# federicomegler/sq-learn

Measured on AMD Instinct MI355X. Metric: q-means fit samples/sec (Lloyd samples*iterations/s, delta-means + tomography noise), higher is better.
Workload: dtype fp32; 1 GPU; model=q-means k=1024 delta=0.5 (10000000 x 256 synthetic), global_batch=10000000, seq_len=256, parallelism=dp1

## Files before the change

sq_learn_amd/csrc/estep_f32.hip:

```cpp
#include "common.h"
#include "band.h"
#include "f16_tile.h"

namespace sq {

constexpr int kMaxCand = 16;

#ifndef SQ_SPLIT_ACC_ALL
#define SQ_SPLIT_ACC_ALL 1
#endif
template <int KSD, int TOP = 2>
__global__ void __launch_bounds__(256, 1) estep_f32_kernel(
    const float* __restrict__ X, const _Float16* __restrict__ C, const float* __restrict__ xn,
    int* __restrict__ labels, float* __restrict__ mind, long long* __restrict__ ovf_rows,
    int* __restrict__ ovf_count, double* __restrict__ part, long long n, int k_pad, float alpha,
    float inv_alpha2, float delta_s, RngKey key, long long row_offset, int ovf_cap,
    const long long* __restrict__ rlist, const int* __restrict__ rcount,
    const float* __restrict__ cmax2_p, long long* __restrict__ mrows, int* __restrict__ mcand,
    int* __restrict__ multi_count, unsigned char* __restrict__ xflag, long long mcap) {
  const float Cm = cmax2_p ? sqrtf(*cmax2_p) * (1.0f + 0x1p-16f) : 0.0f;
  constexpr bool SPLIT_ACC = SQ_SPLIT_ACC_ALL || TOP == 3;
  constexpr float kEps3 =
      SPLIT_ACC ? (3.0f * 0x1p-22f + (KSD * 16 + 18.0f) * 0x1p-24f + 2.0f * KSD * 16 * 0x1p-34f) *
                      1.0625f
// ... 906 lines not shown
  for (int p = 0; p < PER && act; ++p) {
    if (act & (1ull << p)) {
      rlist[pos++] = c0 + (long long)p * 256 + tid;
      act &= ~(1ull << p);
    }
  }
  int mpos = base_m + (ex >> 16);
  for (int p = 0; p < PER && rec; ++p) {
    if (rec & (1ull << p)) {
      mrows[mpos++] = c0 + (long long)p * 256 + tid;
      rec &= ~(1ull << p);
    }
  }
  int bpos = base_b + before_b + incl_b - mine_b;
  for (int p = 0; p < PER && recb; ++p) {
    if (recb & (1ull << p)) {
      mrows_b[bpos++] = c0 + (long long)p * 256 + tid;
      recb &= ~(1ull << p);
    }
  }
}

struct MultiRec {
  GapRec* rec = nullptr;
  int* mflag = nullptr;
  int it_now = 0, it_lo = 0;
  int ring = 0;
  const _Float16* dsh = nullptr;
  const float* dq = nullptr;
  long long dsh_stride = 0;
  long long* mrows_b = nullptr;
  int* count_b = nullptr;
  int* n_done = nullptr;
};
static thread_local MultiRec g_mrec;
struct Ovf2 {
  void* rows = nullptr;
  int* count = nullptr;
};
static thread_local Ovf2 g_ovf2;
extern "C" int sq_set_overflow2(void* rows, void* count) {
  g_ovf2.rows = rows;
  g_ovf2.count = (int*)count;
  return (rows != nullptr) != (count != nullptr) ? (int)hipErrorInvalidValue : 0;
}
extern "C" int sq_multi_records(void* rec, void* mflag, int it_now, int it_lo, int ring,
                                const void* dsh, const void* dq, long long dsh_stride,
                                void* mrows_b, void* count_b, void* n_done) {
  g_mrec.rec = (GapRec*)rec;
  g_mrec.mflag = (int*)mflag;
  g_mrec.it_now = it_now;
  g_mrec.it_lo = it_lo;
  g_mrec.ring = ring;
  g_mrec.dsh = (const _Float16*)dsh;
  g_mrec.dq = (const float*)dq;
  g_mrec.dsh_stride = dsh_stride;
  g_mrec.mrows_b = (long long*)mrows_b;
  g_mrec.count_b = (int*)count_b;
  g_mrec.n_done = (int*)n_done;
  return (rec && (it_now < 1 || it_lo < 1 || it_lo > it_now || ring < 2 || ring > 16 || !mflag ||
                  !dsh || !dq || !mrows_b || !count_b))
             ? (int)hipErrorInvalidValue
             : 0;
}

extern "C" int sq_bounds_filter(const void* labels, void* ub, void* lb, const void* shift,
                                const void* smax, long long n, double delta, void* rlist,
                                void* rcount, const void* mflag, void* mrows, void* multi_count,
                                const void* cc, const void* fidx, int nf, int k, void* stream,
                                void* corr, void* rec_count) {
  if (n <= 0) return 0;
  if (!mflag || !mrows || !multi_count) return (int)hipErrorInvalidValue;
  if (nf < 0 || nf > 64 || (nf > 0 && (!cc || !fidx || k <= nf))) return (int)hipErrorInvalidValue;
  hipStream_t st = (hipStream_t)stream;
  static long long resident = 0;
  if (resident == 0) {
    int dev = 0, cus = 0, per_cu = 0;
    hipGetDevice(&dev);
    hipDeviceGetAttribute(&cus, hipDeviceAttributeMultiprocessorCount, dev);
    hipOccupancyMaxActiveBlocksPerMultiprocessor(&per_cu, (const void*)bounds_filter_kernel<32>,
                                                 256, 0);
    resident = (long long)(cus > 0 ? cus : 256) * (per_cu > 0 ? per_cu : 4);
  }
  auto pick = [&](int per) { return (n + per * 256LL - 1) / (per * 256LL) <= resident; };
  static const int per_env = [] {
    const char* e = getenv("SQ_BF_PER");
    return e ? atoi(e) : 0;
  }();
  int per = pick(8) ? 8 : pick(16) ? 16 : pick(20) ? 20 : pick(32) ? 32 : 64;
  if (per_env == 4 || per_env == 8 || per_env == 16 || per_env == 20 || per_env == 32 ||
      per_env == 64)
    per = per_env;
// ... 376 lines not shown
  acc = __builtin_amdgcn_fdot2(__builtin_bit_cast(gs_h2, a.x), __builtin_bit_cast(gs_h2, b.x), acc,
                               false);
  acc = __builtin_amdgcn_fdot2(__builtin_bit_cast(gs_h2, a.y), __builtin_bit_cast(gs_h2, b.y), acc,
                               false);
  acc = __builtin_amdgcn_fdot2(__builtin_bit_cast(gs_h2, a.z), __builtin_bit_cast(gs_h2, b.z), acc,
                               false);
  acc = __builtin_amdgcn_fdot2(__builtin_bit_cast(gs_h2, a.w), __builtin_bit_cast(gs_h2, b.w), acc,
                               false);
  return acc;
}
__device__ __forceinline__ float gs_dot(const uint2 a, const uint2 b, float acc) {
  acc = __builtin_amdgcn_fdot2(__builtin_bit_cast(gs_h2, a.x), __builtin_bit_cast(gs_h2, b.x), acc,
                               false);
  acc = __builtin_amdgcn_fdot2(__builtin_bit_cast(gs_h2, a.y), __builtin_bit_cast(gs_h2, b.y), acc,
                               false);
  return acc;
}
__device__ __forceinline__ uint4 gs_zero(uint4) { return make_uint4(0u, 0u, 0u, 0u); }
template <int CTRL>
__device__ __forceinline__ float gs_dpp_add(float v) {
  return v + __int_as_float(__builtin_amdgcn_update_dpp(0, __float_as_int(v), CTRL, 0xF, 0xF,
                                                         false));
}
__device__ __forceinline__ uint2 gs_zero(uint2) { return make_uint2(0u, 0u); }

template <int DX>
__global__ void __launch_bounds__(256) gap_screen_kernel(
    const _Float16* __restrict__ Xh, const float* __restrict__ xn,
    const long long* __restrict__ mrows_b, const int* __restrict__ count_b,
    const _Float16* __restrict__ dsh, long long dsh_stride, const float* __restrict__ dq,
    long long dq_stride, float inv_alpha, float delta, int* __restrict__ labels,
    GapRec* __restrict__ rec, int* __restrict__ mflag, int it_now, int ring, int rebase_age,
    long long* __restrict__ mrows, int* __restrict__ multi_count, long long cap,
    int* __restrict__ n_done) {
  constexpr int LPR = 32;
  using VT = typename std::conditional<DX % 256 == 0, uint4, uint2>::type;
  constexpr int HV = (int)sizeof(VT) / 2;
  constexpr int V = DX / (LPR * HV);
  static_assert(DX % 128 == 0 && V >= 1, "gap screen: d_pad multiple of 128");
  const int lane = threadIdx.x & 63;
  const int sub = lane & (LPR - 1);
  const bool hi = lane >= LPR;
  const long long cnt = min((long long)*count_b, cap);
  const long long gw = (long long)blockIdx.x * (blockDim.x >> 6) + (threadIdx.x >> 6);
  const long long nw = (long long)gridDim.x * (blockDim.x >> 6);
  const long long nblk = (cnt + 63) / 64;
  const float sub_err = sqrtf((float)DX) * 0x1p-25f * inv_alpha;
  constexpr float gam = (float)(DX + 16) * 0x1p-24f;
  uint32_t done_cnt = 0;
  auto rl = [](int v, int l) -> int { return __builtin_amdgcn_readlane(v, l); };
  auto rlf = [](float v, int l) -> float {
    return __int_as_float(__builtin_amdgcn_readlane(__float_as_int(v), l));
  };
  for (long long blk = gw; blk < nblk; blk += nw) {
    const long long e = blk * 64 + lane;
    const bool live = e < cnt;
    const long long g = mrows_b[live ? e : cnt - 1];
    const int base_it = mflag[g] - 2;
    const int rslot = base_it % ring, age = it_now - base_it;
    const float4* rp = reinterpret_cast<const float4*>(rec + g);
    const float4 r0 = rp[0], r1 = rp[1];
    const float xq = xn[g];
    const unsigned id0 = __float_as_uint(r1.z), id1 = __float_as_uint(r1.w);
    const int c_r = (int)(id0 >> 30) + 1, slot = (int)((id0 >> 14) & 3u);
    int jc[kGapCand];
    jc[0] = (int)(id0 & 0x3FFFu);
    jc[1] = (int)((id0 >> 16) & 0x3FFFu);
    jc[2] = (int)(id1 & 0x3FFFu);
    jc[3] = (int)((id1 >> 16) & 0x3FFFu);
    const float* dqs = dq + (size_t)rslot * dq_stride;
    float4 d0[kGapCand];
    float inv[kGapCand];
#pragma unroll
    for (int c = 0; c < kGapCand; ++c) {
      d0[c] = reinterpret_cast<const float4*>(dqs)[2 * jc[c]];
      inv[c] = dqs[8 * jc[c] + 4];
    }
    float y[kGapCand] = {0.0f, 0.0f, 0.0f, 0.0f};
    constexpr int NB = 4;
    VT xv[NB][V], sv[NB][kGapCand][V];
    int pcm[NB];
    auto issue = [&](int p, int b) {
// ... 85 lines not shown
    float gm = gn[0];
#pragma unroll
    for (int c = 1; c < kGapCand; ++c)
      if (gn[c] < gm) {
        gm = gn[c];
        m = c;
      }
    bool done = live && c_r >= 2 && slot < c_r && err < 0.25f * delta + 1.0f;
    float gmx = 0.0f;
#pragma unroll
    for (int c = 0; c < kGapCand; ++c)
      if (c < c_r && c != m) {
        done = done && (gn[c] - gm > delta + 2.0f * err);
        gmx = fmaxf(gmx, gn[c]);
      }
    if (done && (m != slot || age >= rebase_age)) {
      const float da_n = da + gm;
      float err_n =
          (m == slot ? err : 2.0f * err) + 0x1p-22f * (gmx + fabsf(da_n) + fabsf(gm));
      err_n *= 1.0f + 0x1p-20f;
      float gr[kGapCand];
#pragma unroll
      for (int c = 0; c < kGapCand; ++c) gr[c] = c < c_r ? gn[c] - gm : 0.0f;
      float4* wp = reinterpret_cast<float4*>(rec + g);
      wp[0] = make_float4(da_n, err_n, gr[0], gr[1]);
      wp[1] = make_float4(gr[2], gr[3],
                          __uint_as_float((id0 & ~(3u << 14)) | (unsigned)m << 14),
                          __uint_as_float(id1));
      if (m != slot) labels[g] = jc[0] * (m == 0) + jc[1] * (m == 1) + jc[2] * (m == 2) +
                                 jc[3] * (m == 3);
      mflag[g] = it_now + 2;
    }
    const bool fwd = live && !done;
    const unsigned long long fm = __ballot(fwd);
    if (fm) {
      int fb = 0;
      if (lane == 0) fb = atomicAdd(multi_count, __popcll(fm));
      fb = __shfl(fb, 0, 64);
      const long long se = (long long)fb + __popcll(fm & ((1ull << lane) - 1ull));
      if (fwd && se < cap) mrows[se] = g;
    }
    done_cnt += __popcll(__ballot(done));
  }
  if (n_done && lane == 0 && done_cnt) atomicAdd(n_done, (int)done_cnt);
}

__global__ void __launch_bounds__(256) shift_operand_kernel(
    const float* __restrict__ Cprev, const float* __restrict__ Cnew, int ldc, int d, int d_pad,
    int k, double alpha, float* __restrict__ snap, _Float16* __restrict__ dsh,
    float* __restrict__ dq, int snew, unsigned valid) {
  const int lane = threadIdx.x & 63;
  const int j = blockIdx.x * 4 + (threadIdx.x >> 6);
  const int sl = blockIdx.y;
  if (j >= k || !((valid >> sl) & 1u)) return;
  const size_t rs = (size_t)sl * k + j;
  const float* cn = Cnew + (size_t)j * ldc;
  float* sn = snap + rs * d_pad;
  const bool fresh = sl == snew;
  const float* co = fresh ? Cprev + (size_t)j * ldc : sn;
  double amax = 0.0;
  for (int f = lane; f < d; f += 64) amax = fmax(amax, fabs((double)cn[f] - (double)co[f]));
#pragma unroll
  for (int o = 32; o > 0; o >>= 1) amax = fmax(amax, __shfl_xor(amax, o, 64));
  int ex2 = 0;
  if (amax > 0.0) frexp(amax, &ex2);
  const double beta = amax > 0.0 ? ldexp(1.0, 14 - ex2) : 1.0;
  double q = 0.0, nrm = 0.0, nd = 0.0, e2 = 0.0;
  for (int f = lane; f < d_pad; f += 64) {
    const float a32 = f < d ? co[f] : 0.0f;
    const double a = (double)a32, b = f < d ? (double)cn[f] : 0.0;
    const double sft = b - a;
    const _Float16 h = (_Float16)(float)(beta * sft);
    dsh[rs * d_pad + f] = h;
    if (fresh) sn[f] = a32;
    const double r = sft - (double)h / beta;
    q += sft * (b + a);
// ... 243 lines not shown
                       (const long long*)rlist, (const int*)rcount, (float*)ub, (float*)lb,
                       (int*)mflag);
  };
  static const bool list_rs1 = [] {
    const char* e = getenv("SQ_X64_LIST_RS1");
    return !(e && e[0] == '0');
  }();
  if (rlist && (list_rs == 1 || (list_rs == 0 && list_rs1)))
    go(std::integral_constant<int, 1>{});
  else
    go(std::integral_constant<int, X64RowSets<KSD>::value>{});
  int rc = (int)hipGetLastError();
  if (rc) return rc;
  const long long rblocks = (n / 16 + 63) / 64;
  const unsigned rgrid = (unsigned)(rblocks < 4096 ? (rblocks > 0 ? rblocks : 1) : 4096);
  if (xflag && g_mrec.rec && ub) {
    if constexpr (KSD * 16 % 128 == 0) {
      static long long gres = 0;
      if (gres == 0) {
        int dev = 0, cus = 0, per_cu = 0;
        hipGetDevice(&dev);
        hipDeviceGetAttribute(&cus, hipDeviceAttributeMultiprocessorCount, dev);
        hipOccupancyMaxActiveBlocksPerMultiprocessor(
            &per_cu, (const void*)gap_screen_kernel<KSD * 16>, 256, 0);
        gres = (long long)(cus > 0 ? cus : 256) * (per_cu > 0 ? per_cu : 2);
      }
      const unsigned bgrid = (unsigned)min(max(rblocks, 1LL), gres);
      hipLaunchKernelGGL(gap_screen_kernel<KSD * 16>, dim3(bgrid), dim3(256), 0, st,
                         (const _Float16*)Xh, (const float*)xn, g_mrec.mrows_b, g_mrec.count_b,
                         g_mrec.dsh, g_mrec.dsh_stride, g_mrec.dq,
                         g_mrec.dsh_stride / (KSD * 16) * 8, 1.0f / alpha, (float)delta,
                         (int*)labels, g_mrec.rec, g_mrec.mflag, g_mrec.it_now, g_mrec.ring,
                         max(1, g_mrec.ring / 2), (long long*)mrows, (int*)multi_count, n,
                         g_mrec.n_done);
    }
  }
  if (xflag) {
    static int sgrid = 0, sil = 0;
    if (sgrid == 0) {
      const char* ei = getenv("SQ_SCREEN_IL");
      sil = ei ? atoi(ei) : 0;
      const char* e = getenv("SQ_SCREEN_GRID");
      sgrid = e ? atoi(e) : 1024;
      if (sgrid <= 0) sgrid = 4096;
    }
    const unsigned fgrid2 = (unsigned)(rblocks < sgrid ? (rblocks > 0 ? rblocks : 1) : sgrid);
    auto fk = ub ? recheck_fast_kernel<KSD * 16, SQ_SCREEN_LPR, true>
                 : recheck_fast_kernel<KSD * 16, SQ_SCREEN_LPR, false>;
    hipLaunchKernelGGL(fk, dim3(fgrid2), dim3(256), 0, st, (const float*)X, (const float*)Cm,
                       (const long long*)mrows, (const int*)mcand, (const int*)multi_count,
                       (int*)labels, (float*)mind, n, delta, (float*)ub, (unsigned char*)xflag,
                       sil, g_mrec.rec, g_mrec.mflag, g_mrec.it_now, key, row_offset,
                       (float*)corr);
  }
  if (!defer_rows)
    hipLaunchKernelGGL(recheck_rows_kernel<KSD * 16>, dim3(rgrid), dim3(256), 0, st,
                       (const float*)X, (const float*)Cm, (const long long*)mrows,
                       (const int*)mcand, (const int*)multi_count, (int*)labels, (float*)mind, n,
                       delta, key, row_offset, (float*)corr, (float*)ub,
                       (const unsigned char*)xflag);
  return (int)hipGetLastError();
}

extern "C" {

int sq_estep_f32(const void* X, const void* C, const void* xn, void* labels, void* mind,
                 void* ovf_rows, void* ovf_count, void* part, int part_cap, void* inertia,
// ... 151 lines not shown
```

sq_learn_amd/csrc/module.cpp:

```cpp
#define PY_SSIZE_T_CLEAN
#include <Python.h>
#include <hip/hip_runtime.h>

extern "C" {
__attribute__((weak)) int sq_trunc_normal_add(void*, int, long long, double, unsigned, unsigned, unsigned, unsigned,
                        unsigned long long, void*);
__attribute__((weak)) int sq_philox_normal(void*, int, long long, double, double, unsigned, unsigned, unsigned, unsigned,
                     unsigned long long, void*);
__attribute__((weak)) int sq_philox_uniform(void*, long long, unsigned, unsigned, unsigned, unsigned, unsigned long long,
                      void*);
__attribute__((weak)) int sq_ae_batch(const void*, const void*, void*, long long, int, unsigned, unsigned, unsigned,
                unsigned, unsigned long long, void*);
__attribute__((weak)) int sq_pe_batch(const void*, const void*, void*, long long, unsigned, unsigned, unsigned, unsigned,
                unsigned long long, void*);
__attribute__((weak)) int sq_tomography(const void*, int, int, const void*, int, int, const void*,
                                        void*, void*, int, unsigned, unsigned, unsigned, unsigned,
                                        long long, void*, double);
__attribute__((weak)) int sq_mnom_segments(const void*, long long, const void*, long long,
                                           long long, const void*, void*, long long, unsigned,
                                           unsigned, unsigned, unsigned, const void*, int, void*);
__attribute__((weak)) int sq_bounds_filter(const void*, void*, void*, const void*, const void*,
                                           long long, double, void*, void*, const void*, void*,
                                           void*, const void*, const void*, int, int, void*, void*,
                                           void*);
__attribute__((weak)) int sq_multi_records(void*, void*, int, int, int, const void*, const void*,
                                           long long, void*, void*, void*);
__attribute__((weak)) int sq_set_overflow2(void*, void*);
__attribute__((weak)) int sq_shift_operand(const void*, const void*, int, int, int, int, double,
                                           void*, void*, void*, int, int, unsigned, void*);
__attribute__((weak)) int sq_fast_centroids(void*, const void*, const void*, int, int, int, void*,
                                            void*, void*, void*);
__attribute__((weak)) int sq_xtx(const void*, int, long long, const void*, int, const void*, int,
                                 long long, const void*, int, long long, int, int, void*, void*,
                                 int, void*);
__attribute__((weak)) int sq_xtx_geometry(int, int, int, int*, int*, int*);
__attribute__((weak)) int sq_xw(const void*, int, long long, const void*, long long, int,
                                const void*, long long, int, int, void*, int, long long, void*);
__attribute__((weak)) int sq_ipe_fused(const void*, long long, const void*, const void*,
                                       const void*, const void*, const void*, void*, void*,
                                       long long, int, int, int, int, double, int, unsigned,
                                       unsigned, unsigned, unsigned, unsigned, unsigned, unsigned,
                                       unsigned, unsigned, unsigned, unsigned, unsigned, long long,
                                       int, void*, void*, void*, const void*, const void*,
                                       long long, const void*, const void*);
__attribute__((weak)) int sq_ipe16(int, const long long*, const double*, void*);
__attribute__((weak)) int sq_kmpp_batch(int, const long long*, void*);
__attribute__((weak)) int sq_centroid_delta(const void*, const void*, const void*, void*, void*,
                                            void*, long long, int, int, int, int, void*, void*,
                                            void*, void*);
__attribute__((weak)) int sq_centroid_delta_lists(const void*, const void*, const void*, void*,
                                                  void*, void*, long long, int, int, int, int,
                                                  void*, void*, void*, const void*, const void*,
                                                  const void*, const void*, const void*,
                                                  const void*, void*);
__attribute__((weak)) int sq_cluster_inertia(const void*, const void*, const void*, const void*,
                                             int, int, int, int, void*, void*);
__attribute__((weak)) int sq_pairwise_reduce(const void*, const void*, void*, int, int, int, int,
                                             double, int, void*);
__attribute__((weak)) int sq_forest_apply(const void*, const void*, const void*, const void*,
// ... 186 lines not shown
  double stop_err = 0.0;
  if (!PyArg_ParseTuple(a, "KiiKiiKKKiIIIILK|d", &V, &r, &d, &sched, &T, &mode, &first, &err, &out,
                        &ninf, &k0, &k1, &s0, &s1, &roff, &st, &stop_err))
    return nullptr;
  CHECK(sq_tomography)
  return ret(sq_tomography(P(V), r, d, P(sched), T, mode, P(first), P(err), P(out), ninf, k0, k1,
                           s0, s1, roff, P(st), stop_err));
}

static PyObject* py_mnom_segments(PyObject*, PyObject* a) {
  unsigned long long W, wrow, Ns, cnt, sid, st; long long ldw, m, B, ldc; int level;
  unsigned k0, k1, s0, s1;
  if (!PyArg_ParseTuple(a, "KLKLLKKLIIIIKiK", &W, &ldw, &wrow, &m, &B, &Ns, &cnt, &ldc, &k0, &k1,
                        &s0, &s1, &sid, &level, &st))
    return nullptr;
  CHECK(sq_mnom_segments)
  return ret(sq_mnom_segments(P(W), ldw, P(wrow), m, B, P(Ns), P(cnt), ldc, k0, k1, s0, s1, P(sid),
                              level, P(st)));
}

static PyObject* py_bounds_filter(PyObject*, PyObject* a) {
  unsigned long long lab, ub, lb, sh, sm, rl, rc, mf, mr, mcnt, cc, fi, st, mc = 0, rcn = 0;
  long long n;
  double delta; int nf, k;
  if (!PyArg_ParseTuple(a, "KKKKKLdKKKKKKKiiK|KK", &lab, &ub, &lb, &sh, &sm, &n, &delta, &rl, &rc,
                        &mf, &mr, &mcnt, &cc, &fi, &nf, &k, &st, &mc, &rcn))
    return nullptr;
  CHECK(sq_bounds_filter)
  return ret(sq_bounds_filter(P(lab), P(ub), P(lb), P(sh), P(sm), n, delta, P(rl), P(rc), P(mf),
                              P(mr), P(mcnt), P(cc), P(fi), nf, k, P(st), P(mc), P(rcn)));
}

static PyObject* py_multi_records(PyObject*, PyObject* a) {
  unsigned long long rec, mf, dsh, dq, mb, cb, nd; int now, lo, ring; long long ds;
  if (!PyArg_ParseTuple(a, "KKiiiKKLKKK", &rec, &mf, &now, &lo, &ring, &dsh, &dq, &ds, &mb, &cb,
                        &nd))
    return nullptr;
  CHECK(sq_multi_records)
  return ret(sq_multi_records(P(rec), P(mf), now, lo, ring, P(dsh), P(dq), ds, P(mb), P(cb),
                              P(nd)));
}

static PyObject* py_set_overflow2(PyObject*, PyObject* a) {
  unsigned long long rows, cnt;
  if (!PyArg_ParseTuple(a, "KK", &rows, &cnt)) return nullptr;
  CHECK(sq_set_overflow2)
  return ret(sq_set_overflow2(P(rows), P(cnt)));
}

static PyObject* py_shift_operand(PyObject*, PyObject* a) {
  unsigned long long co, cn, snap, dsh, dq, st; int ldc, d, dp, k, ring, snew; double alpha;
  unsigned valid;
  if (!PyArg_ParseTuple(a, "KKiiiidKKKiiIK", &co, &cn, &ldc, &d, &dp, &k, &alpha, &snap, &dsh,
                        &dq, &ring, &snew, &valid, &st))
    return nullptr;
  CHECK(sq_shift_operand)
  return ret(sq_shift_operand(P(co), P(cn), ldc, d, dp, k, alpha, P(snap), P(dsh), P(dq), ring,
                              snew, valid, P(st)));
}

static PyObject* py_fast_centroids(PyObject*, PyObject* a) {
  unsigned long long sh, sq, C, idx, smr, cc, st; int k, d, nf;
  if (!PyArg_ParseTuple(a, "KKKiiiKKKK", &sh, &sq, &C, &k, &d, &nf, &idx, &smr, &cc, &st))
    return nullptr;
  CHECK(sq_fast_centroids)
  return ret(sq_fast_centroids(P(sh), P(sq), P(C), k, d, nf, P(idx), P(smr), P(cc), P(st)));
}

static PyObject* py_centroid_delta(PyObject*, PyObject* a) {
  unsigned long long X, lab, prev, sums, cnts, q, h, c, pm, st; long long n; int d, k, xe, qe;
  if (!PyArg_ParseTuple(a, "KKKKKKLiiiiKKKK", &X, &lab, &prev, &sums, &cnts, &q, &n, &d, &k, &xe,
                        &qe, &h, &c, &pm, &st))
    return nullptr;
// ... 534 lines not shown
```

sq_learn_amd/models/cluster/_lloyd.py:

```python

import math
import os

import torch

from ...runtime.rng import RngKey
from ...ops import kmeans as K
from ...ops import linalg as L
from ...ops.random import trunc_normal_add_
from ...ops.failure import failure_inject_
from ...ops import _native as nat
from ...parallel.comm import Comm
from ...utils import tracing


class _HostScalars:

    __slots__ = ("host", "event", "sink")

    def __init__(self, host, event, sink=None):
        self.host, self.event, self.sink = host, event, sink

    def tolist(self):
        self.event.synchronize()
# ... 108 lines not shown
            self.perm2 = torch.empty(max(4 * self.n, 1), dtype=torch.int32, device=dev)
            self.buf.corr = torch.zeros(max(self.n, 1), dtype=torch.float32, device=dev)
            nr = int(self._nrows_global)
            self.qexp = K.fixed_point_exp(self._max_abs ** 2 * self.dm, nr)
        self.inc_valid = False
        self.bounds = (self.certified
                       and os.environ.get("SQ_ESTEP_BOUNDS", "1") != "0")
        self.keep_max = float(os.environ.get("SQ_ESTEP_KEEP_MAX", "0.8"))
        self.probe_every = 2
        self._kept_frac = None
        self._kept_prev = None
        self._skips = 0
        self._probing = False
        self._filter_ran = False
        self._minus1 = torch.full((1,), -1, dtype=torch.int32, device=dev)
        if self.bounds:
            self.ub = torch.zeros(max(self.n, 1), dtype=torch.float32, device=dev)
            self.lb = torch.zeros(max(self.n, 1), dtype=torch.float32, device=dev)
            self.rlist = torch.empty(max(self.n, 1), dtype=torch.int64, device=dev)
            self.rcount = torch.zeros(1, dtype=torch.int32, device=dev)
            self.shift_s = torch.zeros(self.k, dtype=torch.float64, device=dev)
            self.smax = torch.zeros(1, dtype=torch.float64, device=dev)
            self.n_fast = min(int(os.environ.get("SQ_ESTEP_FAST", "16")), self.k - 1)
            self.fast_idx = torch.zeros(max(self.n_fast, 1), dtype=torch.int32, device=dev)
            self.fast_cc = torch.zeros(max(self.k * (self.n_fast + 1), 1), dtype=torch.float32,
                                       device=dev)
        self.mrec = None
        mr = os.environ.get("SQ_MULTI_RECORDS", "auto")
        if (self.bounds and self.incremental and self.d_pad % 128 == 0 and self.k <= 16384
                and (mr == "1" or (mr == "auto" and self.n >= 4_000_000))):
            R = min(max(int(os.environ.get("SQ_GAP_RING", "8")), 2), 16)
            self.mrec = torch.zeros((max(self.n, 1), 8), dtype=torch.float32, device=dev)
            self.rows_b = torch.empty(max(self.n, 1), dtype=torch.int64, device=dev)
            self.gsnap = torch.zeros((R, self.k, self.d_pad), dtype=torch.float32, device=dev)
            self.dsh = torch.zeros((R, self.k, self.d_pad), dtype=torch.float16, device=dev)
            self.dq = torch.zeros((R, self.k, 8), dtype=torch.float32, device=dev)
            self._rit = 2
            self._rlo = 2
        self.bounds_valid = False

    def _prepare_reduce(self):
        dev = self.device
        self.dm = self.Xm.shape[1]
        self.buf = K.EStepBuffers(self.n, dev)
        mx = torch.stack([self.Xm.abs().max().float() if self.n else torch.zeros((), device=dev),
                          (self.sample_weight.abs().max().float() if self.sample_weight is not None
                           and self.n else torch.zeros((), device=dev))]).double()
        nrows = torch.full((1,), float(self.n), dtype=torch.float64, device=dev)
        self.comm.all_reduce_(mx, op="max")
        self.comm.all_reduce_(nrows)
        mxl = mx.tolist()
        self._max_abs, self._nrows_global = mxl[0], nrows.item()
        self.rws = K.ReduceWorkspace(self.n, self.k, dev).set_scale(
            mxl[0], int(nrows.item()), mxl[1] if self.sample_weight is not None else None)
        self.sums = torch.zeros((self.k, self.dm), dtype=torch.float64, device=dev)
        self.counts = torch.zeros(self.k, dtype=torch.float64, device=dev)
        self.packed = torch.zeros(self.k * self.d + self.k + 1, dtype=torch.float64, device=dev)
        self.shift = torch.zeros(1, dtype=torch.float64, device=dev)
        self.shift_part = torch.zeros(self.k, dtype=torch.float64, device=dev)
        self.C = torch.zeros((self.k, self.d), dtype=torch.float32, device=dev)
        self.C_new = torch.zeros_like(self.C)
        self.cn = torch.full((self.k_pad,), K.BIG, dtype=torch.float32, device=dev)
        self.scalars = torch.zeros(4, dtype=torch.float64, device=dev)
        self.scalars[3] = -1.0
        self.weights = (self.sample_weight.to(torch.float32).contiguous()
                        if self.sample_weight is not None else None)
# ... 98 lines not shown
            self.cn.copy_(d["cn"].to(self.device))

    def estep(self, C=None):
        self._pending = None
        if C is not None:
            self.set_centers(C)
        lab, mind, inertia = self._estep(self._key("band_select"), full=True)
        if self.fast and self.C_op is not None and self.certified:
            K.fill_mind_native(self.Xf32, self.C, lab, mind)
            K.sum_f32_native(mind, self.n, self.mind_part, self.buf.inertia)
        return lab, mind, inertia

    def _estep(self, key, full=False):
        self._dlists = None
        if self.fast and self.C_op is not None and self.certified:
            with tracing.range("estep_x64"):
                Cp = self.C if self.d == self.d_pad else self._padded_centers()
                rows = None
                self._filter_ran = False
                if self.bounds and not full:
                    mode = self._filter_mode()
                    if mode == "filter" and not self.bounds_valid:
                        mode = "bounds"
                else:
                    mode = "bounds" if self.bounds else "none"
                self._bounds_kept = mode != "none"
                screen = (self.incremental and not full
                          and os.environ.get("SQ_SCREEN", "1") != "0")
                if self.mrec is not None and screen:
                    K.ensure_multi_buffers(self.buf, self.n, self.device, True)
                    R = self.dsh.shape[0]
                    K.multi_records(self.mrec, self.buf.mflag, self._rit,
                                    max(self._rlo, self._rit - R + 1), self.dsh, self.dq,
                                    self.rows_b, self.buf.counts[5:6], self.buf.counts[4:5])
                else:
                    K.multi_records(None)
                try:
                    probe = mode == "filter" and self._probing
                    zero = True
                    if mode == "filter":
                        self._filter_ran = True
                        K.ensure_multi_buffers(self.buf, self.n, self.device, True)
                        self.rcount = self.buf.counts[3:4]
                        self.buf.counts.zero_()
                        K.bounds_filter_native(self.buf.labels[:self.n], self.ub, self.lb,
                                               self.shift_s, self.smax, self.delta, self.rlist,
                                               self.rcount, self.buf, cc=self.fast_cc,
                                               nf=self.n_fast, fidx=self.fast_idx)
                        if probe:
                            self.buf.counts[:3].zero_()
                            self.buf.counts[5:6].zero_()
                        else:
                            rows = (self.rlist, self.rcount)
                            self._dlists = ((self.rlist, self.rcount),
                                            (self.buf.multi_rows, self.buf.counts[7:8]),
                                            (self.rows_b, self.buf.counts[5:6])
                                            if self.mrec is not None and screen else None)
                        zero = False
                    lab, mind = K.estep_x64_native(self.Xh16, self.Xf32, self.C_op, Cp, self.xn,
                                                   self.cmax2, self.k, self.delta, self.alpha, key,
                                                   self.row_offset, self.buf,
                                                   bounds=(self.ub, self.lb)
                                                   if self.bounds and self._bounds_kept else None,
                                                   rows=rows, zero_counts=zero, screen=screen,
                                                   list_rs=self._list_rs())
                finally:
                    if self.mrec is not None:
                        K.multi_records(None)
                if self.mrec is not None and not screen:
                    self._records_epoch()
            return lab, mind, self.buf.inertia
        if self.fast and self.C_op is not None:
            with tracing.range("estep_f32"):
                lab, mind = K.estep_f32_native(self.Xf32, self.C_op, self.xn, self.C, self.k,
                                               self.delta, self.alpha, key, self.row_offset,
                                               self.buf)
            return lab, mind, self.buf.inertia
        if self.fast:
            with tracing.range("estep_bf16"):
                lab, mind = K.estep_native(self.Xb, self.C_bf16, self.cn, self.xn, self.k,
                                           self.delta, key, self.row_offset, self.buf)
            return lab, mind, self.buf.inertia
        if self.ipe:
            return self._estep_ipe(key)
        return self._estep_generic(key)

    def _filter_mode(self):
        sd = getattr(self, "_sc_dev", None)
        if sd is not None:
# ... 111 lines not shown
            C32 = self.C.float().contiguous()
            cn = (C32 * C32).sum(1).contiguous()
            with tracing.range("ipe_fused"):
                K.ipe_fused_native(self.Xf, K.ipe_center_fragments(C32, kp, dp), self._ipe_xn, cn,
                                   self.k, kp, dp, eps, self.ipe_Q, ipe_key,
                                   self._key("band_select"), self.row_offset, labels32, mind,
                                   C=C32, hint_labels=hint, skip_key=self._key("ipe_skip"),
                                   stats=getattr(self, "ipe_stats", None))
            return labels32, mind, mind.double().sum().reshape(1)
        if self.device.type == "cuda":
            n = self.n
            labels32 = torch.empty(n, dtype=torch.int32, device=self.device)
            mind = torch.empty(n, dtype=torch.float32, device=self.device)
            C32 = self.C.float()
            cn = (C32 * C32).sum(1).contiguous()
            step = max(256, min(self._chunk_rows(), 1 << 16))
            for s in range(0, n, step):
                e = min(n, s + step)
                G = self.Xf[s:e].float() @ C32.T
                K.ipe_estep_native(G, self.xn[s:e].float().contiguous(), cn, eps, self.ipe_Q,
                                   ipe_key, self.row_offset + s, labels32[s:e], mind[s:e])
            return labels32, mind, mind.double().sum().reshape(1)
        lab, mind = K.ipe_estep_torch(self.Xf, self.C, eps, ipe_key, self.row_offset, self.k_pad,
                                      Q=self.ipe_Q)
        return lab, mind, mind.double().sum().reshape(1)

    def _noise_bound(self):
        if not self.intermediate_error or self.delta <= 0 or self.true_tomography:
            return 0.0
        return (self.delta / 2.0) / math.sqrt(self.k * self.d)

    def mstep(self, labels, inertia, events=None):
        noise_key = self._key("trunc_normal")
        if self.fast and getattr(self, "incremental", False) and self.buf.corr is not None:
            return self._mstep_incremental(labels, inertia, noise_key, events)
        if self.fast:
            with tracing.range("mstep"):
                exact = self.C_op is not None and self.certified
                Cold = None
                if exact:
                    Cold = self.C if self.dm == self.d else self._padded_centers()
                in_pass = exact and self.dm <= 256
                K.centroid_reduce_native(self.Xm, labels, self.weights, self.sums,
                                         self.counts, self.k, self.rws,
                                         mind=self.buf.mind if in_pass else None,
                                         C_old=Cold if in_pass else None)
                if exact and not in_pass:
                    K.fill_mind_native(self.Xf32, self.C, labels, self.buf.mind)
                if exact:
                    K.sum_f32_native(self.buf.mind, self.n, self.mind_part, inertia)
                sums = self.sums if self.dm == self.d else self.sums[:, :self.d].contiguous()
                K.pack_stats_native(sums, self.counts, inertia, self.packed, self.k, self.d,
                                    self.rws, weighted=self.weights is not None)
            if events is not None:
                events[0].record()
            with tracing.range("allreduce"):
                self.comm.all_reduce_(self.packed)
            if events is not None:
                events[1].record()
            self._last_counts = self.packed[self.k * self.d:self.k * self.d + self.k]
            with tracing.range("finalize"):
                K.centroid_finalize_native(self.packed, self.C, self.C_new, self.C_bf16, self.cn,
                                           self.shift, self.k, self.d, self._noise_bound(),
                                           noise_key, self.empty_policy,
                                           shift_part=self.shift_part, scalars=self.scalars,
                                           buf=self.buf, C_f16=self.C_op, alpha=self.alpha,
                                           k_pad=self.k_pad,
# ... 47 lines not shown
            packed = torch.cat([sums.reshape(-1).double(), counts.double(),
                                inertia.double().reshape(1)])
        self.comm.all_reduce_(packed)
        kd = self.k * self.d
        sums = packed[:kd].reshape(self.k, self.d)
        counts = packed[kd:kd + self.k]
        self._last_counts = counts
        self._C_prev = self.C
        tot_inertia = packed[-1]
        old = self.C
        new = torch.where(counts[:, None] > 0, sums / counts[:, None],
                          old.double() if self.empty_policy == 0 else torch.zeros_like(sums))
        new = new.to(old.dtype).contiguous()
        b = self._noise_bound()
        if b > 0:
            flat = new.view(-1)
            trunc_normal_add_(flat, b, noise_key, offset=0)
        self.C = new
        if self.intermediate_error and self.true_tomography and self.delta > 0:
            self._true_tomography_centers()
        dd = self.C.double() - old.double()
        shift = (dd * dd).sum()
        return torch.stack([tot_inertia, shift, torch.zeros((), dtype=torch.float64,
                                                            device=self.device)])

    def _mstep_incremental(self, labels, inertia, noise_key, events):
        with tracing.range("mstep_incremental"):
            if not self.inc_valid:
                self.sums.zero_()
                self.counts.zero_()
                self.qsum.zero_()
                self.prev_labels.fill_(-1)
            dl = os.environ.get("SQ_DELTA_LISTS")
            use = (self.n <= 4_000_000) if dl is None else dl != "0"
            lists = getattr(self, "_dlists", None) if (use and self.inc_valid
                                                       and not self.failure_prob > 0) else None
            self._dlists = None
            if lists is not None:
                self.delta_list_steps = getattr(self, "delta_list_steps", 0) + 1
            K.centroid_delta_native(self.Xm, labels, self.prev_labels, self.sums, self.counts,
                                    self.qsum, self.k, self.rws, self.perm2, self.qexp,
                                    lists=lists)
            self.inc_valid = True
            Cold = self.C if self.dm == self.d else self._padded_centers()
            if self.dm == self.d:
                K.mstep_stats_native(self.sums, self.counts, self.qsum, Cold, self.k, self.dm,
                                     self.rws, self.qexp, self.buf.corr, self.n, self.mind_part,
                                     inertia, self.packed)
            else:
                K.cluster_inertia_native(self.sums, self.counts, self.qsum, Cold, self.k, self.dm,
                                         self.rws, self.qexp, self.mind_part[512:512 + self.k])
                K.sum_f32_native(self.buf.corr, self.n, self.mind_part, inertia, extra=self.k)
                K.pack_stats_native(self.sums[:, :self.d].contiguous(), self.counts, inertia,
                                    self.packed, self.k, self.d, self.rws, weighted=False)
        if events is not None:
            events[0].record()
        with tracing.range("allreduce"):
            self.comm.all_reduce_(self.packed)
        if events is not None:
            events[1].record()
        self._last_counts = self.packed[self.k * self.d:self.k * self.d + self.k]
        with tracing.range("finalize"):
            K.centroid_finalize_native(self.packed, self.C, self.C_new, self.C_bf16, self.cn,
                                       self.shift, self.k, self.d, self._noise_bound(),
                                       noise_key, self.empty_policy,
                                       shift_part=self.shift_part, scalars=self.scalars,
                                       buf=self.buf, C_f16=self.C_op, alpha=self.alpha,
# ... 118 lines not shown
        else:
            labels, mind, inertia = self._estep(self._key("band_select"))
        if self.failure_prob > 0:
            extra = {}
            if self.fast and getattr(self, "bounds", False):
                extra["lb"] = self.lb
            if self.fast and self.C_op is not None and self.certified:
                Cm = self.C if self.dm == self.d else self._padded_centers()
                extra.update(X=self.Xm, C=Cm, mind=self.buf.mind)
                if getattr(self, "incremental", False) and self.buf.corr is not None:
                    extra["corr"] = self.buf.corr
            failure_inject_(labels, self.k, self.failure_prob, self.failure_attempts,
                            self._key("failure"), self.row_offset, self.failure_counters, **extra)
        sc = self.mstep(labels, inertia)
        if self.relocate_empty:
            counts = self._last_counts
            ne = (counts == 0).sum().to(torch.float64).reshape(1)
            vals = torch.cat([sc.reshape(-1)[:3].to(torch.float64), ne]).cpu()
            if vals[3] > 0:
                self._undo_update()
                labels = self._relocate(labels, counts.clone())
                sc = self.mstep(labels, inertia)
                vals = torch.cat([sc.reshape(-1)[:3].to(torch.float64),
                                  torch.zeros(1, dtype=torch.float64, device=sc.device)]).cpu()
            sc = vals
        self.it += 1
        if self.pipeline and self.fast and not self.relocate_empty:
            if self._sc_ring is None:
                self._sc_ring = [(torch.empty(sc.numel(), dtype=sc.dtype, pin_memory=True),
                                  torch.cuda.Event()) for _ in range(2)]
            host, ev = self._sc_ring[self.it & 1]
            host.copy_(sc.reshape(-1), non_blocking=True)
            ev.record()
            if self._label_snap is None or self._label_snap.shape != labels.shape:
                self._label_snap = torch.empty_like(labels)
            self._label_snap.copy_(labels)
            labels = self._label_snap
            self._pending = self._estep(self._key("band_select"))
            sc = _HostScalars(host, ev, self._on_scalars)
        elif getattr(self, "bounds", False) and torch.is_tensor(sc) and sc.numel() > 3:
            self._sc_dev = sc
        return labels, sc
```

sq_learn_amd/ops/kmeans.py:

```python

import math
import os

import numpy as np

import torch

from ..runtime.rng import RngKey, philox4x32, MASK32
from . import _native as nat
from .random import amplitude_estimation_batch

FAST_D = (16, 32, 64, 128, 256)
X64_D = FAST_D + (384, 512, 640, 768, 896, 1024)
X64_MAX_K = 16384
BIG = 3.0e38


def pad_features(d):
    for f in X64_D:
        if d <= f:
            return f
    return ((d + 15) // 16) * 16


# ... 95 lines not shown
def ipe_estep_torch(X, C, eps, key, row_offset, k_pad, Q=13, chunk_rows=256):
    n, k = X.shape[0], C.shape[0]
    labels = torch.empty(n, dtype=torch.int64)
    mind = torch.empty(n, dtype=torch.float64)
    cn = (C.double() ** 2).sum(1)
    for s in range(0, n, chunk_rows):
        e = min(n, s + chunk_rows)
        xb = X[s:e].double()
        xn = (xb * xb).sum(1)
        G = xb @ C.double().T
        S = xn[:, None] + cn[None, :]
        a = (S - 2 * G) / (2 * S)
        a = torch.where(a.abs() <= 1e-15, torch.zeros_like(a), a)
        eps_a = eps * torch.clamp(G.abs(), min=1.0) / S
        at = amplitude_estimation_batch(a.clamp(0, 1), eps_a, key, Q=Q,
                                        offset=(row_offset + s) * k)
        sv = S * (1 - 2 * at) / 2
        Dt = xn[:, None] + cn[None, :] - 2 * sv
        g = torch.arange(s, e, dtype=torch.int64) + row_offset
        lab, mn = band_select_torch(Dt, g, 0.0, key, k_pad, tie_only=True)
        labels[s:e] = lab
        mind[s:e] = mn
    return labels, mind


class EStepBuffers:

    def __init__(self, n, device, ovf_cap=None):
        self.labels = torch.empty(n, dtype=torch.int32, device=device)
        self.mind = torch.empty(n, dtype=torch.float32, device=device)
        self.ovf_cap = int(ovf_cap if ovf_cap is not None else max(n, 1))
        self.ovf_rows = torch.empty(self.ovf_cap, dtype=torch.int64, device=device)
        self.ovf_thr = torch.empty(self.ovf_cap, dtype=torch.float32, device=device)
        self.counts = torch.zeros(8, dtype=torch.int32, device=device)
        self.ovf2_rows = None
        self.exact_flag = None
        self.ovf_count = self.counts[0:1]
        self.dense_rows = None
        self.multi_rows = None
        self.multi_cand = None
        self.mflag = None
        self.corr = None
        self.ovf_clean = True
        self.inertia = torch.zeros(1, dtype=torch.float64, device=device)
        self.part_cap = n // 32 + 64
        self.inertia_part = torch.zeros(self.part_cap, dtype=torch.float64, device=device)


def estep_native(Xb, C_bf16, cn, xn, k, delta, key: RngKey, row_offset, buf: EStepBuffers,
                 stream=None):
    n, d_pad = Xb.shape
    k_pad = C_bf16.shape[0] * 64
    assert Xb.dtype == torch.bfloat16 and C_bf16.dtype == torch.bfloat16
    assert tuple(C_bf16.shape[1:]) == (d_pad // 8 + 2, 64, 8) and d_pad in FAST_D
    assert Xb.is_contiguous() and C_bf16.is_contiguous() and cn.is_contiguous()
    assert buf.labels.numel() >= n and buf.part_cap >= 8
    st = stream if stream is not None else nat.stream_handle(Xb.device)
    m = nat.native()
    if not buf.ovf_clean:
        buf.ovf_count.zero_()
    buf.ovf_clean = False
    m.estep_bf16(Xb.data_ptr(), C_bf16.data_ptr(), buf.inertia_part.data_ptr(), buf.ovf_thr.data_ptr(),
                 xn.data_ptr(), buf.labels.data_ptr(), buf.mind.data_ptr(), buf.ovf_rows.data_ptr(),
                 buf.ovf_count.data_ptr(), buf.inertia.data_ptr(), n, d_pad, k, k_pad,
                 float(delta), int(buf.part_cap), key.k0, key.k1, key.s0, key.s1, int(row_offset),
                 buf.ovf_cap, st)
    m.band_select_rows(Xb.data_ptr(), C_bf16.data_ptr(), buf.ovf_thr.data_ptr(), xn.data_ptr(),
# ... 128 lines not shown
    assert ub.dtype == torch.float32 and lb.dtype == torch.float32 and rlist.numel() >= n
    assert shift.dtype == torch.float64 and smax.dtype == torch.float64
    assert buf.mflag is not None and buf.mflag.numel() >= n
    rc = nat.native().bounds_filter(labels.data_ptr(), ub.data_ptr(), lb.data_ptr(),
                                    shift.data_ptr(), smax.data_ptr(), n, float(delta),
                                    rlist.data_ptr(), rcount.data_ptr(), buf.mflag.data_ptr(),
                                    buf.multi_rows.data_ptr(), buf.counts[2:3].data_ptr(),
                                    0 if cc is None else cc.data_ptr(),
                                    0 if cc is None else fidx.data_ptr(),
                                    int(nf if cc is not None else 0), int(shift.numel()),
                                    nat.stream_handle(labels.device),
                                    0 if buf.corr is None else buf.corr.data_ptr(),
                                    buf.counts[7:8].data_ptr())
    if rc:
        raise RuntimeError(f"bounds_filter failed (hip error {rc})")


def fast_centroids_native(shift, C, nf, idx, smax_rest, cc, shift_sq=None):
    k, d = C.shape
    assert C.dtype == torch.float32 and C.is_contiguous() and shift.dtype == torch.float64
    assert 0 <= nf < k and idx.numel() >= nf and cc.numel() >= k * (nf + 1)
    assert shift.numel() >= k and shift.is_contiguous()
    if shift_sq is not None:
        assert shift_sq.dtype == torch.float64 and shift_sq.is_contiguous() and shift_sq.numel() >= k
    rc = nat.native().fast_centroids(shift.data_ptr(),
                                     0 if shift_sq is None else shift_sq.data_ptr(), C.data_ptr(),
                                     k, d, int(nf), idx.data_ptr(), smax_rest.data_ptr(),
                                     cc.data_ptr(), nat.stream_handle(C.device))
    if rc:
        raise RuntimeError(f"fast_centroids failed (hip error {rc})")


def multi_records(rec=None, mflag=None, it_now=0, it_lo=0, dsh=None, dq=None, rows_b=None,
                  count_b=None, n_done=None):
    if rec is None:
        nat.native().multi_records(0, 0, 0, 0, 0, 0, 0, 0, 0, 0, 0)
        return
    assert rec.dtype == torch.float32 and rec.shape[-1] == 8 and mflag.dtype == torch.int32
    assert dsh.dtype == torch.float16 and dq.dtype == torch.float32 and rows_b.dtype == torch.int64
    assert dsh.dim() == 3 and dq.shape[:2] == dsh.shape[:2] and dq.shape[2] == 8
    rc = nat.native().multi_records(rec.data_ptr(), mflag.data_ptr(), int(it_now), int(it_lo),
                                    int(dsh.shape[0]), dsh.data_ptr(), dq.data_ptr(),
                                    int(dsh.stride(0)), rows_b.data_ptr(), count_b.data_ptr(),
                                    0 if n_done is None else n_done.data_ptr())
    if rc:
        raise RuntimeError(f"multi_records failed (hip error {rc})")


def shift_operand_native(C_prev, C_new, alpha, snap, dsh, dq, snew, valid):
    k, d = C_new.shape[0], C_new.shape[1]
    ring, _, d_pad = dsh.shape
    assert C_prev.dtype == torch.float32 and C_new.dtype == torch.float32
    assert C_prev.stride() == C_new.stride() and C_new.stride(1) == 1
    assert tuple(snap.shape) == (ring, k, d_pad) and tuple(dq.shape) == (ring, k, 8)
    rc = nat.native().shift_operand(C_prev.data_ptr(), C_new.data_ptr(), int(C_new.stride(0)), int(d),
                                    int(d_pad), int(k), float(alpha), snap.data_ptr(), dsh.data_ptr(),
                                    dq.data_ptr(), int(ring), int(snew), int(valid),
                                    nat.stream_handle(C_new.device))
    if rc:
        raise RuntimeError(f"shift_operand failed (hip error {rc})")


def ensure_multi_buffers(buf: EStepBuffers, n, device, bounds=False):
    if buf.dense_rows is None or buf.dense_rows.numel() < n:
        buf.dense_rows = torch.empty(max(n, 1), dtype=torch.int64, device=device)
    if buf.multi_rows is None or buf.multi_rows.numel() < n:
        buf.multi_rows = torch.empty(max(n, 1), dtype=torch.int64, device=device)
        buf.multi_cand = torch.empty((max(n, 1), 17), dtype=torch.int32, device=device)
    if bounds and (buf.mflag is None or buf.mflag.numel() < n):
        buf.mflag = torch.zeros(max(n, 1), dtype=torch.int32, device=device)


def centroid_delta_native(X, labels, prev, sums, counts, qsum, k, ws: ReduceWorkspace, perm2,
                          qexp, lists=None):
    n, d = X.shape
    assert X.dtype == torch.float32 and X.is_contiguous() and d % 4 == 0 and d <= 1024
    assert labels.dtype == torch.int32 and prev.dtype == torch.int32 and perm2.numel() >= 4 * n
# ... 869 lines not shown
```

Measured before the change: 13.82 billion samples*iter/s.

## Emit moved-row list from gap screen to drive incremental M-step delta lists

The gap-screen kernel now builds a second row list holding rows that were forwarded or whose label changed, and stages both lists in per-wave LDS buffers so atomics and global writes happen in batches. The incremental M-step's delta lists now use this narrower moved-row list instead of every screened row, and delta lists are enabled for large n whenever multi-records are active. The label snapshot copy is skipped when the incremental M-step ran. This aims to cut M-step work on unchanged rows and to reduce atomic contention, at the cost of extra LDS use and a second list write.

```diff
diff --git a/sq_learn_amd/csrc/estep_f32.hip b/sq_learn_amd/csrc/estep_f32.hip
--- a/sq_learn_amd/csrc/estep_f32.hip
+++ b/sq_learn_amd/csrc/estep_f32.hip
@@ -962,6 +962,8 @@
   long long* mrows_b = nullptr;
   int* count_b = nullptr;
   int* n_done = nullptr;
+  long long* mrows_mv = nullptr;
+  int* count_mv = nullptr;
 };
 static thread_local MultiRec g_mrec;
 struct Ovf2 {
@@ -976,7 +978,8 @@
 }
 extern "C" int sq_multi_records(void* rec, void* mflag, int it_now, int it_lo, int ring,
                                 const void* dsh, const void* dq, long long dsh_stride,
-                                void* mrows_b, void* count_b, void* n_done) {
+                                void* mrows_b, void* count_b, void* n_done, void* mrows_mv,
+                                void* count_mv) {
   g_mrec.rec = (GapRec*)rec;
   g_mrec.mflag = (int*)mflag;
   g_mrec.it_now = it_now;
@@ -988,6 +991,9 @@
   g_mrec.mrows_b = (long long*)mrows_b;
   g_mrec.count_b = (int*)count_b;
   g_mrec.n_done = (int*)n_done;
+  g_mrec.mrows_mv = (long long*)mrows_mv;
+  g_mrec.count_mv = (int*)count_mv;
+  if ((mrows_mv != nullptr) != (count_mv != nullptr)) return (int)hipErrorInvalidValue;
   return (rec && (it_now < 1 || it_lo < 1 || it_lo > it_now || ring < 2 || ring > 16 || !mflag ||
                   !dsh || !dq || !mrows_b || !count_b))
              ? (int)hipErrorInvalidValue
@@ -1430,7 +1436,7 @@
     long long dq_stride, float inv_alpha, float delta, int* __restrict__ labels,
     GapRec* __restrict__ rec, int* __restrict__ mflag, int it_now, int ring, int rebase_age,
     long long* __restrict__ mrows, int* __restrict__ multi_count, long long cap,
-    int* __restrict__ n_done) {
+    int* __restrict__ n_done, long long* __restrict__ mrows_mv, int* __restrict__ count_mv) {
   constexpr int LPR = 32;
   using VT = typename std::conditional<DX % 256 == 0, uint4, uint2>::type;
   constexpr int HV = (int)sizeof(VT) / 2;
@@ -1446,6 +1452,27 @@
   const float sub_err = sqrtf((float)DX) * 0x1p-25f * inv_alpha;
   constexpr float gam = (float)(DX + 16) * 0x1p-24f;
   uint32_t done_cnt = 0;
+  constexpr int kGapStage = 256;
+  __shared__ long long stage_fw[4][kGapStage], stage_mv[4][kGapStage];
+  int n_fw = 0, n_mv = 0;
+  auto flush = [&](const long long* buf, int& cnt, long long* __restrict__ dst, int* counter) {
+    if (cnt == 0) return;
+    int b = 0;
+    if (lane == 0) b = atomicAdd(counter, cnt);
+    b = __shfl(b, 0, 64);
+    __builtin_amdgcn_wave_barrier();
+    for (int i = lane; i < cnt; i += 64)
+      if ((long long)b + i < cap) dst[(long long)b + i] = buf[i];
+    cnt = 0;
+  };
+  auto stage = [&](bool pred, long long row, long long* buf, int& cnt, long long* __restrict__ dst,
+                   int* counter) {
+    const unsigned long long pm = __ballot(pred);
+    if (pm == 0) return;
+    if (cnt + 64 > kGapStage) flush(buf, cnt, dst, counter);
+    if (pred) buf[cnt + __popcll(pm & ((1ull << lane) - 1ull))] = row;
+    cnt += __popcll(pm);
+  };
   auto rl = [](int v, int l) -> int { return __builtin_amdgcn_readlane(v, l); };
   auto rlf = [](float v, int l) -> float {
     return __int_as_float(__builtin_amdgcn_readlane(__float_as_int(v), l));
@@ -1597,16 +1624,13 @@
       mflag[g] = it_now + 2;
     }
     const bool fwd = live && !done;
-    const unsigned long long fm = __ballot(fwd);
-    if (fm) {
-      int fb = 0;
-      if (lane == 0) fb = atomicAdd(multi_count, __popcll(fm));
-      fb = __shfl(fb, 0, 64);
-      const long long se = (long long)fb + __popcll(fm & ((1ull << lane) - 1ull));
-      if (fwd && se < cap) mrows[se] = g;
-    }
+    stage(fwd, g, stage_fw[threadIdx.x >> 6], n_fw, mrows, multi_count);
+    if (mrows_mv)
+      stage(fwd || (done && m != slot), g, stage_mv[threadIdx.x >> 6], n_mv, mrows_mv, count_mv);
     done_cnt += __popcll(__ballot(done));
   }
+  flush(stage_fw[threadIdx.x >> 6], n_fw, mrows, multi_count);
+  if (mrows_mv) flush(stage_mv[threadIdx.x >> 6], n_mv, mrows_mv, count_mv);
   if (n_done && lane == 0 && done_cnt) atomicAdd(n_done, (int)done_cnt);
 }
 
@@ -1916,7 +1940,7 @@
                          g_mrec.dsh_stride / (KSD * 16) * 8, 1.0f / alpha, (float)delta,
                          (int*)labels, g_mrec.rec, g_mrec.mflag, g_mrec.it_now, g_mrec.ring,
                          max(1, g_mrec.ring / 2), (long long*)mrows, (int*)multi_count, n,
-                         g_mrec.n_done);
+                         g_mrec.n_done, g_mrec.mrows_mv, g_mrec.count_mv);
     }
   }
   if (xflag) {
diff --git a/sq_learn_amd/csrc/module.cpp b/sq_learn_amd/csrc/module.cpp
--- a/sq_learn_amd/csrc/module.cpp
+++ b/sq_learn_amd/csrc/module.cpp
@@ -24,7 +24,7 @@
                                            void*, const void*, const void*, int, int, void*, void*,
                                            void*);
 __attribute__((weak)) int sq_multi_records(void*, void*, int, int, int, const void*, const void*,
-                                           long long, void*, void*, void*);
+                                           long long, void*, void*, void*, void*, void*);
 __attribute__((weak)) int sq_set_overflow2(void*, void*);
 __attribute__((weak)) int sq_shift_operand(const void*, const void*, int, int, int, int, double,
                                            void*, void*, void*, int, int, unsigned, void*);
@@ -277,13 +277,13 @@
 }
 
 static PyObject* py_multi_records(PyObject*, PyObject* a) {
-  unsigned long long rec, mf, dsh, dq, mb, cb, nd; int now, lo, ring; long long ds;
-  if (!PyArg_ParseTuple(a, "KKiiiKKLKKK", &rec, &mf, &now, &lo, &ring, &dsh, &dq, &ds, &mb, &cb,
-                        &nd))
+  unsigned long long rec, mf, dsh, dq, mb, cb, nd, mv, cmv; int now, lo, ring; long long ds;
+  if (!PyArg_ParseTuple(a, "KKiiiKKLKKKKK", &rec, &mf, &now, &lo, &ring, &dsh, &dq, &ds, &mb, &cb,
+                        &nd, &mv, &cmv))
     return nullptr;
   CHECK(sq_multi_records)
   return ret(sq_multi_records(P(rec), P(mf), now, lo, ring, P(dsh), P(dq), ds, P(mb), P(cb),
-                              P(nd)));
+                              P(nd), P(mv), P(cmv)));
 }
 
 static PyObject* py_set_overflow2(PyObject*, PyObject* a) {
diff --git a/sq_learn_amd/models/cluster/_lloyd.py b/sq_learn_amd/models/cluster/_lloyd.py
--- a/sq_learn_amd/models/cluster/_lloyd.py
+++ b/sq_learn_amd/models/cluster/_lloyd.py
@@ -164,6 +164,7 @@
             R = min(max(int(os.environ.get("SQ_GAP_RING", "8")), 2), 16)
             self.mrec = torch.zeros((max(self.n, 1), 8), dtype=torch.float32, device=dev)
             self.rows_b = torch.empty(max(self.n, 1), dtype=torch.int64, device=dev)
+            self.rows_moved = torch.empty(max(self.n, 1), dtype=torch.int64, device=dev)
             self.gsnap = torch.zeros((R, self.k, self.d_pad), dtype=torch.float32, device=dev)
             self.dsh = torch.zeros((R, self.k, self.d_pad), dtype=torch.float16, device=dev)
             self.dq = torch.zeros((R, self.k, 8), dtype=torch.float32, device=dev)
@@ -328,7 +329,8 @@
                     R = self.dsh.shape[0]
                     K.multi_records(self.mrec, self.buf.mflag, self._rit,
                                     max(self._rlo, self._rit - R + 1), self.dsh, self.dq,
-                                    self.rows_b, self.buf.counts[5:6], self.buf.counts[4:5])
+                                    self.rows_b, self.buf.counts[5:6], self.buf.counts[4:5],
+                                    self.rows_moved, self.buf.counts[8:9])
                 else:
                     K.multi_records(None)
                 try:
@@ -350,7 +352,7 @@
                             rows = (self.rlist, self.rcount)
                             self._dlists = ((self.rlist, self.rcount),
                                             (self.buf.multi_rows, self.buf.counts[7:8]),
-                                            (self.rows_b, self.buf.counts[5:6])
+                                            (self.rows_moved, self.buf.counts[8:9])
                                             if self.mrec is not None and screen else None)
                         zero = False
                     lab, mind = K.estep_x64_native(self.Xh16, self.Xf32, self.C_op, Cp, self.xn,
@@ -528,7 +530,9 @@
 
     def mstep(self, labels, inertia, events=None):
         noise_key = self._key("trunc_normal")
+        self._mstep_inc = False
         if self.fast and getattr(self, "incremental", False) and self.buf.corr is not None:
+            self._mstep_inc = True
             return self._mstep_incremental(labels, inertia, noise_key, events)
         if self.fast:
             with tracing.range("mstep"):
@@ -642,7 +646,8 @@
                 self.qsum.zero_()
                 self.prev_labels.fill_(-1)
             dl = os.environ.get("SQ_DELTA_LISTS")
-            use = (self.n <= 4_000_000) if dl is None else dl != "0"
+            use = ((self.n <= 4_000_000 or self.mrec is not None) if dl is None
+                   else dl != "0")
             lists = getattr(self, "_dlists", None) if (use and self.inc_valid
                                                        and not self.failure_prob > 0) else None
             self._dlists = None
@@ -827,10 +832,13 @@
             host, ev = self._sc_ring[self.it & 1]
             host.copy_(sc.reshape(-1), non_blocking=True)
             ev.record()
-            if self._label_snap is None or self._label_snap.shape != labels.shape:
-                self._label_snap = torch.empty_like(labels)
-            self._label_snap.copy_(labels)
-            labels = self._label_snap
+            if getattr(self, "_mstep_inc", False):
+                labels = self.prev_labels[:self.n]
+            else:
+                if self._label_snap is None or self._label_snap.shape != labels.shape:
+                    self._label_snap = torch.empty_like(labels)
+                self._label_snap.copy_(labels)
+                labels = self._label_snap
             self._pending = self._estep(self._key("band_select"))
             sc = _HostScalars(host, ev, self._on_scalars)
         elif getattr(self, "bounds", False) and torch.is_tensor(sc) and sc.numel() > 3:
diff --git a/sq_learn_amd/ops/kmeans.py b/sq_learn_amd/ops/kmeans.py
--- a/sq_learn_amd/ops/kmeans.py
+++ b/sq_learn_amd/ops/kmeans.py
@@ -151,7 +151,7 @@
         self.ovf_cap = int(ovf_cap if ovf_cap is not None else max(n, 1))
         self.ovf_rows = torch.empty(self.ovf_cap, dtype=torch.int64, device=device)
         self.ovf_thr = torch.empty(self.ovf_cap, dtype=torch.float32, device=device)
-        self.counts = torch.zeros(8, dtype=torch.int32, device=device)
+        self.counts = torch.zeros(12, dtype=torch.int32, device=device)
         self.ovf2_rows = None
         self.exact_flag = None
         self.ovf_count = self.counts[0:1]
@@ -346,17 +346,22 @@
 
 
 def multi_records(rec=None, mflag=None, it_now=0, it_lo=0, dsh=None, dq=None, rows_b=None,
-                  count_b=None, n_done=None):
+                  count_b=None, n_done=None, rows_moved=None, count_moved=None):
     if rec is None:
-        nat.native().multi_records(0, 0, 0, 0, 0, 0, 0, 0, 0, 0, 0)
+        nat.native().multi_records(0, 0, 0, 0, 0, 0, 0, 0, 0, 0, 0, 0, 0)
         return
     assert rec.dtype == torch.float32 and rec.shape[-1] == 8 and mflag.dtype == torch.int32
     assert dsh.dtype == torch.float16 and dq.dtype == torch.float32 and rows_b.dtype == torch.int64
     assert dsh.dim() == 3 and dq.shape[:2] == dsh.shape[:2] and dq.shape[2] == 8
+    if rows_moved is not None:
+        assert rows_moved.dtype == torch.int64 and rows_moved.numel() >= rows_b.numel()
+        assert count_moved.dtype == torch.int32
     rc = nat.native().multi_records(rec.data_ptr(), mflag.data_ptr(), int(it_now), int(it_lo),
                                     int(dsh.shape[0]), dsh.data_ptr(), dq.data_ptr(),
                                     int(dsh.stride(0)), rows_b.data_ptr(), count_b.data_ptr(),
-                                    0 if n_done is None else n_done.data_ptr())
+                                    0 if n_done is None else n_done.data_ptr(),
+                                    0 if rows_moved is None else rows_moved.data_ptr(),
+                                    0 if rows_moved is None else count_moved.data_ptr())
     if rc:
         raise RuntimeError(f"multi_records failed (hip error {rc})")
 
```

After: 14.78 billion samples*iter/s, median of 6. +6.9%, better.
